# google-deepmind/open_spiel

Measured on AMD Instinct MI355X. Metric: env-steps/sec (batched LegalActions+ApplyAction+status, connect_four), higher is better.
Workload: dtype u64; 1 GPU; connect_four fused LegalActions+ApplyAction+status, 2^20 states/GPU, seed 0x5EED; states_per_gpu=1048576, parallelism=1 independent shard(s), no collective

## Files before the change

open_spiel_amd/csrc/osg_playout.hip:

```cpp
#include <algorithm>

#include "osg_batch_internal.h"

namespace {

template <class G>
__global__ void __launch_bounds__(kBlock)
k_random_steps(typename G::Params p, typename G::word_t* base, int64_t n, uint64_t seed, int64_t index_offset,
               int steps, unsigned long long* partials) {
  __shared__ unsigned long long s_sum[2][kBlock / 64];
  unsigned long long applied = 0, episodes = 0;
  const int64_t stride = static_cast<int64_t>(gridDim.x) * kBlock;
  for (int64_t i = static_cast<int64_t>(blockIdx.x) * kBlock + threadIdx.x; i < n; i += stride) {
    typename G::State s = G::load(p, base, n, i);
    Rng rng(seed, static_cast<uint64_t>(index_offset + i), 0);
    for (int t = 0; t < steps; ++t) {
      if (G::terminal(p, s)) {
        s = G::initial(p);
        ++episodes;
      }
      auto m = G::legal(p, s);
      int a = sample_action<G>(p, s, m, G::current_player(p, s), rng);
      G::apply(p, s, a);
      ++applied;
    }
    G::store(p, base, n, i, s);
  }
  unsigned long long a = applied, e = episodes;
#pragma unroll
  for (int off = 32; off >= 1; off >>= 1) {
    a += __shfl_xor(a, off);
    e += __shfl_xor(e, off);
  }
  if ((threadIdx.x & 63) == 0) {
    s_sum[0][threadIdx.x >> 6] = a;
    s_sum[1][threadIdx.x >> 6] = e;
  }
  __syncthreads();
  if (threadIdx.x == 0) {
    unsigned long long ta = 0, te = 0;
    for (int w = 0; w < kBlock / 64; ++w) { ta += s_sum[0][w]; te += s_sum[1][w]; }
    const int slot = blockIdx.x & (kCounterSlots - 1);
    atomicAdd(&partials[2 * slot], ta);
    atomicAdd(&partials[2 * slot + 1], te);
  }
}
__global__ void __launch_bounds__(64) k_fold_counters(unsigned long long* partials, unsigned long long* counters) {
  const int lane = threadIdx.x;
  unsigned long long a = partials[2 * lane], e = partials[2 * lane + 1];
  partials[2 * lane] = 0;
  partials[2 * lane + 1] = 0;
#pragma unroll
  for (int off = 32; off >= 1; off >>= 1) {
    a += __shfl_xor(a, off);
    e += __shfl_xor(e, off);
  }
  if (lane == 0) {
    counters[0] += a;
    counters[1] += e;
  }
}

constexpr uint64_t kSynthSub = 0x53594E5448ULL;
constexpr int kSynthMaxAttempts = 1 << 14;
template <class G>
__global__ void __launch_bounds__(kBlock)
k_synth(typename G::Params p, typename G::word_t* base, int64_t n, uint64_t seed, int64_t index_offset, int depth_mod,
        uint8_t* actions, int32_t* depth_out) {
  const int64_t i = static_cast<int64_t>(blockIdx.x) * kBlock + threadIdx.x;
  if (i >= n) return;
  Rng rng(seed, static_cast<uint64_t>(index_offset + i), kSynthSub);
  int depth = static_cast<int>(rng.below(static_cast<uint32_t>(depth_mod)));
  typename G::State s = G::initial(p);
  int t = 0, attempt = 0;
  for (;;) {
    const bool term = G::terminal(p, s);
    if (t == depth || term) {
      if (!term) break;
      if (++attempt >= kSynthMaxAttempts) { s = G::initial(p); depth = 0; break; }
      s = G::initial(p);
      t = 0;
      continue;
    }
    const auto m = G::legal(p, s);
    G::apply(p, s, sample_action<G>(p, s, m, G::current_player(p, s), rng));
    ++t;
  }
  G::store(p, base, n, i, s);
  const auto m = G::legal(p, s);
  const int a = sample_action<G>(p, s, m, G::current_player(p, s), rng);
  if (actions) actions[i] = static_cast<uint8_t>(a);
  if (depth_out) depth_out[i] = depth;
}

template <class G>
__global__ void __launch_bounds__(kBlock)
k_rollout(typename G::Params p, const typename G::word_t* base, int64_t n, int num_players, uint64_t seed,
          int64_t index_offset, int n_rollouts, int group, double* sum_returns, int32_t* steps_out) {
  const int64_t total = n * group;
  const int64_t stride = static_cast<int64_t>(gridDim.x) * kBlock;
  int64_t item = static_cast<int64_t>(blockIdx.x) * kBlock + threadIdx.x;
  if (item >= total) return;
  int64_t root = item / group;
  int r = static_cast<int>(item - root * group);
  typename G::State s = G::load(p, base, n, root);
  Rng rng(seed, static_cast<uint64_t>(index_offset + root), static_cast<uint64_t>(r));
  double acc[kMaxPlayers];
#pragma unroll
  for (int q = 0; q < kMaxPlayers; ++q) acc[q] = 0.0;
  int plies = 0, ply = 0;
  for (;;) {
    if (G::terminal(p, s) || ply >= kMaxPlayoutPlies) {
      double ret[kMaxPlayers];
      G::returns(p, s, ret);
#pragma unroll
      for (int q = 0; q < kMaxPlayers; ++q)
        if (q < num_players) acc[q] += ret[q];
      r += group;
      if (r >= n_rollouts) {
#pragma unroll
        for (int q = 0; q < kMaxPlayers; ++q) {
          if (q < num_players) sum_returns[item * num_players + q] = acc[q];
          acc[q] = 0.0;
        }
        if (steps_out) steps_out[item] = plies;
        plies = 0;
        item += stride;
        if (item >= total) break;
        root = item / group;
        r = static_cast<int>(item - root * group);
      }
      s = G::load(p, base, n, root);
      rng = Rng(seed, static_cast<uint64_t>(index_offset + root), static_cast<uint64_t>(r));
      ply = 0;
      continue;
    }
    auto m = G::legal(p, s);
    int a = sample_action<G>(p, s, m, G::current_player(p, s), rng);
    G::apply(p, s, a);
    ++plies;
    ++ply;
  }
}

template <class G>
__global__ void __launch_bounds__(kBlock)
k_rollout_hexfill(typename G::Params p, const typename G::word_t* base, int64_t n, uint64_t seed, int64_t index_offset,
                  int n_rollouts, int group, double* sum_returns) {
  const int64_t total = n * group;
  const int64_t stride = static_cast<int64_t>(gridDim.x) * kBlock;
  for (int64_t item = static_cast<int64_t>(blockIdx.x) * kBlock + threadIdx.x; item < total; item += stride) {
    const int64_t root = item / group;
    const typename G::State s = G::load(p, base, n, root);
    double acc = 0.0;
    for (int r = static_cast<int>(item - root * group); r < n_rollouts; r += group) {
      if (G::terminal(p, s)) {
        acc += G::result(s) == 1 ? 1.0 : -1.0;
        continue;
      }
      Rng rng(seed, static_cast<uint64_t>(index_offset + root), static_cast<uint64_t>(r));
      acc += G::fill_playout_winner(p, s, rng) == 0 ? 1.0 : -1.0;
    }
    sum_returns[item * 2] = acc;
    sum_returns[item * 2 + 1] = -acc + 0.0;
  }
}

template <class G>
void launch_rollout_hexfill(const typename G::Params& p, const void* words, int64_t n, uint64_t seed, int64_t index_offset,
                            int n_rollouts, int group, double* d_part, unsigned blocks, hipStream_t st) {
  if constexpr (is_hex<G>::value)
    k_rollout_hexfill<G><<<dim3(blocks), dim3(kBlock), 0, st>>>(p, static_cast<const typename G::word_t*>(words), n, seed,
                                                              index_offset, n_rollouts, group, d_part);
}

__global__ void __launch_bounds__(kBlock)
k_rollout_fold(const double* __restrict__ part, const int32_t* __restrict__ part_steps, int64_t n, int num_players,
               int group, double* __restrict__ sum_returns, int32_t* __restrict__ steps_out) {
  const int64_t k = static_cast<int64_t>(blockIdx.x) * kBlock + threadIdx.x;
  if (k >= n * num_players) return;
  const int64_t root = k / num_players;
  const int q = static_cast<int>(k - root * num_players);
  double v = 0.0;
  for (int j = 0; j < group; ++j) v += part[(root * group + j) * num_players + q];
  sum_returns[k] = v;
  if (steps_out && q == 0) {
    int32_t t = 0;
    for (int j = 0; j < group; ++j) t += part_steps[root * group + j];
    steps_out[root] = t;
  }
}

}

extern "C" {

int osg_random_steps(osg_batch* b, uint64_t seed, int64_t index_offset, int steps, unsigned long long* d_counters) {
  osg_ctx* ctx = b->ctx;
  unsigned long long* partials = ctx->d_illegal + 1;
  int64_t blocks = (b->n + kBlock - 1) / kBlock;
  constexpr int64_t kMaxBlocks = 4096;
  if (blocks > kMaxBlocks) blocks = kMaxBlocks;
  if (int rc = for_game(b->spec, [&](auto g, const auto& P) {
        using G = typename decltype(g)::type;
        k_random_steps<G><<<dim3(static_cast<unsigned>(blocks)), dim3(kBlock), 0, ctx->stream>>>(P,
            static_cast<typename G::word_t*>(b->words()), b->n, seed, index_offset,
            steps, partials);
        return OSG_OK;
      })) return rc;
  k_fold_counters<<<dim3(1), dim3(64), 0, ctx->stream>>>(partials, d_counters);
  OSG_HIP(hipGetLastError());
  return OSG_OK;
}

int osg_synth_batch(osg_batch* b, uint64_t seed, int64_t index_offset, int depth_mod, uint8_t* d_actions,
                    int32_t* d_depth) {
  if (!b) return set_error(OSG_ERR_INVALID, "osg_synth_batch: null batch");
  if (depth_mod < 1 || depth_mod > b->spec.desc.max_game_length)
    return set_error(OSG_ERR_INVALID, "osg_synth_batch: depth_mod must lie in [1, MaxGameLength()]");
  if (int rc = refuse_endless_playouts(b->spec, "osg_synth_batch")) return rc;
  if (d_actions && b->spec.desc.num_distinct_actions > 255)
    return set_error(OSG_ERR_UNSUPPORTED, "osg_synth_batch: d_actions holds one byte per action; pass NULL for games with more "
                                          "than 255 actions");
  osg_ctx* ctx = b->ctx;
  if (int rc = for_game(b->spec, [&](auto g, const auto& P) {
        using G = typename decltype(g)::type;
        k_synth<G><<<dim3(grid_for(b->n)), dim3(kBlock), 0, ctx->stream>>>(P,
            static_cast<typename G::word_t*>(b->words()), b->n, seed, index_offset, depth_mod,
            d_actions, d_depth);
        return OSG_OK;
      })) return rc;
  OSG_HIP(hipGetLastError());
  return OSG_OK;
}

int osg_rollout(const osg_batch* roots, uint64_t seed, int64_t index_offset, int n_rollouts, double* sum_returns,
                int32_t* steps, int on_host) {
  osg_ctx* ctx = roots->ctx;
  const int P_ = roots->spec.desc.num_players;
  const int64_t n = roots->n;
  if (n_rollouts <= 0) return set_error(OSG_ERR_INVALID, "n_rollouts must be positive");
  if (int rc = refuse_endless_playouts(roots->spec, "osg_rollout")) return rc;
  constexpr int kLanesLog2 = 19;
  int64_t group = ((int64_t{1} << kLanesLog2) + n - 1) / std::max<int64_t>(n, 1);
  if (group > n_rollouts) group = n_rollouts;
  if (group < 1) group = 1;
  const size_t ret_bytes = sizeof(double) * P_ * n, step_bytes = sizeof(int32_t) * n;
  const size_t off_steps = align_up(ret_bytes), off_part = on_host ? align_up(off_steps + step_bytes) : 0;
  const size_t part_bytes = group > 1 ? ret_bytes * group : 0, off_part_steps = align_up(off_part + part_bytes);
  const size_t scratch_bytes = group > 1 ? off_part_steps + step_bytes * group : (on_host ? off_steps + step_bytes : 0);
  char* scratch = nullptr;
  if (scratch_bytes) {
    void* ptr;
    int rc = osg_ctx_scratch(ctx, scratch_bytes, &ptr);
    if (rc) return rc;
    scratch = static_cast<char*>(ptr);
  }
  double* d_sum = on_host ? reinterpret_cast<double*>(scratch) : sum_returns;
  int32_t* d_steps = steps ? (on_host ? reinterpret_cast<int32_t*>(scratch + off_steps) : steps) : nullptr;
  double* d_part = group > 1 ? reinterpret_cast<double*>(scratch + off_part) : d_sum;
  int32_t* d_part_steps = d_steps ? (group > 1 ? reinterpret_cast<int32_t*>(scratch + off_part_steps) : d_steps) : nullptr;
  const int64_t total = n * group;
  int64_t blocks = (total + kBlock - 1) / kBlock;
  if (blocks > 2048) blocks = 2048;
  if (!steps && roots->spec.desc.game_kind == kHex) {
    if (int rc = for_game(roots->spec, [&](auto g, const auto& P) {
          using G = typename decltype(g)::type;
          launch_rollout_hexfill<G>(P, roots->words(), n, seed, index_offset, n_rollouts,
              static_cast<int>(group), d_part, static_cast<unsigned>(blocks), ctx->stream);
          return OSG_OK;
        })) return rc;
  } else {
  if (int rc = for_game(roots->spec, [&](auto g, const auto& P) {
        using G = typename decltype(g)::type;
        k_rollout<G><<<dim3(static_cast<unsigned>(blocks)), dim3(kBlock), 0, ctx->stream>>>(P,
            static_cast<const typename G::word_t*>(roots->words()), n, P_, seed,
            index_offset, n_rollouts, static_cast<int>(group), d_part,
            d_part_steps);
        return OSG_OK;
      })) return rc;
  }
  if (group > 1)
    k_rollout_fold<<<dim3(grid_for(n * P_)), dim3(kBlock), 0, ctx->stream>>>(d_part, d_part_steps, n, P_,
                                                                             static_cast<int>(group), d_sum, d_steps);
  OSG_HIP(hipGetLastError());
  if (on_host) {
    OSG_HIP(hipMemcpyAsync(sum_returns, d_sum, ret_bytes, hipMemcpyDeviceToHost, ctx->stream));
    if (steps) OSG_HIP(hipMemcpyAsync(steps, d_steps, step_bytes, hipMemcpyDeviceToHost, ctx->stream));
    OSG_HIP(hipStreamSynchronize(ctx->stream));
  }
  return OSG_OK;
}

}
```

Baseline: 256.1 billion env-steps/s.

## Add specialized connect-four random-walk kernel with mover/opponent bitboards and kth-open table

Adds a dedicated connect_four playout kernel for the standard variant. It keeps the state as mover/opponent 32-bit bitboard halves plus an open-column mask, resets terminal states branchlessly, and picks the k-th open column from a shared-memory lookup table. This replaces the generic legal/sample/apply path and is meant to remove per-step legal-mask construction and generic action sampling. In exchange it adds a separate code path that must stay consistent with the generic state encoding and RNG semantics.

```diff
diff --git a/open_spiel_amd/csrc/osg_playout.hip b/open_spiel_amd/csrc/osg_playout.hip
--- a/open_spiel_amd/csrc/osg_playout.hip
+++ b/open_spiel_amd/csrc/osg_playout.hip
@@ -1,6 +1,7 @@
 #include <algorithm>
 
 #include "osg_batch_internal.h"
+#include "step/osg_c4_walk.h"
 
 namespace {
 
@@ -45,6 +46,49 @@
     atomicAdd(&partials[2 * slot + 1], te);
   }
 }
+__global__ void __launch_bounds__(kBlock)
+k_random_steps_c4std(uint64_t* base, int64_t n, uint64_t seed, int64_t index_offset, int steps,
+                     unsigned long long* partials) {
+  __shared__ unsigned long long s_sum[2][kBlock / 64];
+  __shared__ uint8_t s_kth[kC4KthOpenBytes];
+  for (int e = threadIdx.x; e < kC4KthOpenBytes; e += kBlock) s_kth[e] = static_cast<uint8_t>(c4_kth_open_entry(e));
+  __syncthreads();
+  unsigned long long applied = 0, episodes = 0;
+  const int64_t stride = static_cast<int64_t>(gridDim.x) * kBlock;
+  for (int64_t i = static_cast<int64_t>(blockIdx.x) * kBlock + threadIdx.x; i < n; i += stride) {
+    C4Walk s = c4_walk_load(base[i], base[n + i]);
+    Rng rng(seed, static_cast<uint64_t>(index_offset + i), 0);
+    uint32_t resets = 0;
+#pragma unroll 2
+    for (int t = 0; t < steps; ++t) {
+      resets += c4_walk_reset(s);
+      const uint32_t k = rng.below(static_cast<uint32_t>(__builtin_popcount(s.open)));
+      c4_walk_move(s, c4_kth_open(s_kth, s.open, k));
+    }
+    base[i] = c4_walk_pack0(s);
+    base[n + i] = c4_walk_pack1(s);
+    episodes += resets;
+    applied += static_cast<unsigned long long>(steps > 0 ? steps : 0);
+  }
+  unsigned long long a = applied, e = episodes;
+#pragma unroll
+  for (int off = 32; off >= 1; off >>= 1) {
+    a += __shfl_xor(a, off);
+    e += __shfl_xor(e, off);
+  }
+  if ((threadIdx.x & 63) == 0) {
+    s_sum[0][threadIdx.x >> 6] = a;
+    s_sum[1][threadIdx.x >> 6] = e;
+  }
+  __syncthreads();
+  if (threadIdx.x == 0) {
+    unsigned long long ta = 0, te = 0;
+    for (int w = 0; w < kBlock / 64; ++w) { ta += s_sum[0][w]; te += s_sum[1][w]; }
+    const int slot = blockIdx.x & (kCounterSlots - 1);
+    atomicAdd(&partials[2 * slot], ta);
+    atomicAdd(&partials[2 * slot + 1], te);
+  }
+}
 __global__ void __launch_bounds__(64) k_fold_counters(unsigned long long* partials, unsigned long long* counters) {
   const int lane = threadIdx.x;
   unsigned long long a = partials[2 * lane], e = partials[2 * lane + 1];
@@ -201,7 +245,10 @@
   int64_t blocks = (b->n + kBlock - 1) / kBlock;
   constexpr int64_t kMaxBlocks = 4096;
   if (blocks > kMaxBlocks) blocks = kMaxBlocks;
-  if (int rc = for_game(b->spec, [&](auto g, const auto& P) {
+  if (b->spec.desc.game_kind == kC4 && b->spec.c4_std) {
+    k_random_steps_c4std<<<dim3(static_cast<unsigned>(blocks)), dim3(kBlock), 0, ctx->stream>>>(
+        static_cast<uint64_t*>(b->words()), b->n, seed, index_offset, steps, partials);
+  } else if (int rc = for_game(b->spec, [&](auto g, const auto& P) {
         using G = typename decltype(g)::type;
         k_random_steps<G><<<dim3(static_cast<unsigned>(blocks)), dim3(kBlock), 0, ctx->stream>>>(P,
             static_cast<typename G::word_t*>(b->words()), b->n, seed, index_offset,
diff --git a/open_spiel_amd/csrc/step/osg_c4_walk.h b/open_spiel_amd/csrc/step/osg_c4_walk.h
--- /dev/null
+++ b/open_spiel_amd/csrc/step/osg_c4_walk.h
@@ -0,0 +1,87 @@
+#ifndef OSG_C4_WALK_H_
+#define OSG_C4_WALK_H_
+
+#include "osg_c4_step_split.h"
+
+namespace osg {
+
+struct C4Walk {
+  uint32_t m_lo, m_hi;
+  uint32_t t_lo, t_hi;
+  uint32_t flags;
+  uint32_t stones;
+  uint32_t open;
+};
+
+OSG_HD C4Walk c4_walk_load(uint64_t w0, uint64_t w1) {
+  C4Walk s;
+  const uint32_t x_lo = static_cast<uint32_t>(w0), x_hi = static_cast<uint32_t>(w0 >> 32) & 0x00FFFFFFu;
+  const uint32_t o_lo = static_cast<uint32_t>(w1), o_hi = static_cast<uint32_t>(w1 >> 32);
+  s.flags = static_cast<uint32_t>(w0 >> 56);
+  const uint32_t all_lo = x_lo | o_lo, all_hi = x_hi | o_hi;
+  s.stones = static_cast<uint32_t>(__builtin_popcount(all_lo) + __builtin_popcount(all_hi));
+  s.open = c4_open_columns(all_lo, all_hi);
+  const bool odd = (s.stones & 1u) != 0u;
+  s.m_lo = odd ? o_lo : x_lo;
+  s.m_hi = odd ? o_hi : x_hi;
+  s.t_lo = odd ? x_lo : o_lo;
+  s.t_hi = odd ? x_hi : o_hi;
+  return s;
+}
+OSG_HD uint64_t c4_walk_pack0(const C4Walk& s) {
+  const bool odd = (s.stones & 1u) != 0u;
+  const uint32_t lo = odd ? s.t_lo : s.m_lo, hi = odd ? s.t_hi : s.m_hi;
+  return (static_cast<uint64_t>(hi | (s.flags << 24)) << 32) | lo;
+}
+OSG_HD uint64_t c4_walk_pack1(const C4Walk& s) {
+  const bool odd = (s.stones & 1u) != 0u;
+  const uint32_t lo = odd ? s.m_lo : s.t_lo, hi = odd ? s.m_hi : s.t_hi;
+  return (static_cast<uint64_t>(hi) << 32) | lo;
+}
+
+OSG_HD uint32_t c4_walk_reset(C4Walk& s) {
+  const uint32_t over = s.flags & 1u;
+  const uint32_t keep = over - 1u;
+  s.m_lo &= keep;
+  s.m_hi &= keep;
+  s.t_lo &= keep;
+  s.t_hi &= keep;
+  s.stones &= keep;
+  s.open |= ~keep & 0x7Fu;
+  return over;
+}
+
+constexpr int kC4KthOpenBytes = 128 * 8;
+OSG_HD uint32_t c4_kth_open_entry(uint32_t index) {
+  const uint32_t mask = index >> 3, k = index & 7u;
+  uint32_t seen = 0, col = 7u;
+  for (uint32_t c = 0; c < 7u; ++c) {
+    if (!((mask >> c) & 1u)) continue;
+    if (seen == k) col = c;
+    ++seen;
+  }
+  return col;
+}
+OSG_HD uint32_t c4_kth_open(const uint8_t* table, uint32_t mask, uint32_t k) { return table[(mask << 3) | k]; }
+
+OSG_HD void c4_walk_move(C4Walk& s, uint32_t col) {
+  const uint32_t sh = col * 7u;
+  const uint32_t all_lo = s.m_lo | s.t_lo, all_hi = s.m_hi | s.t_hi;
+  const uint32_t cells = static_cast<uint32_t>(((static_cast<uint64_t>(all_hi) << 32) | all_lo) >> sh);
+  const uint32_t cell = (cells + 1u) & 0x3Fu;
+  const uint64_t put = static_cast<uint64_t>(cell) << sh;
+  const uint32_t b_lo = s.m_lo | static_cast<uint32_t>(put), b_hi = s.m_hi | static_cast<uint32_t>(put >> 32);
+  s.open ^= (cell >> 5) << col;
+  const uint32_t mover = s.stones & 1u;
+  s.stones += 1u;
+  const bool win = c4_has_four(b_lo, b_hi);
+  const bool done = win | (s.stones == 42u);
+  s.flags = done ? (((win ? mover : 2u) << 1) | 1u) : 0u;
+  s.m_lo = s.t_lo;
+  s.m_hi = s.t_hi;
+  s.t_lo = b_lo;
+  s.t_hi = b_hi;
+}
+
+}
+#endif
```

Measured after the change: 255.7 billion env-steps/s. About the same (-0.2%).
